# zyc-123/InstanceDiff

Measured on AMD Instinct MI355X. Metric: denoising steps/sec (256x256 bs16), higher is better.
Workload: dtype f32; 1 GPU; 256x256 1-ch synthetic, 1000-step reverse chain, batch 16 per GPU, 2 UNet fwd + reverse update per step; global_batch=16, parallelism=replicas x1 (no collective)

## Files before the change

include/idiff.h:

```cpp
#ifndef IDIFF_H
#define IDIFF_H

#include <stdint.h>

#ifdef __cplusplus
extern "C" {
#endif

#define IDIFF_OK 0
#define IDIFF_E_BADARG (-1)
#define IDIFF_E_UNSUPPORTED (-2)
#define IDIFF_E_HIP (-3)

typedef void* idiff_stream_t;

const char* idiff_last_error(void);
int idiff_version(void);
int64_t idiff_launch_count(void);
int idiff_device_info(int* num_cu, int* wave_size, char* arch_name, int arch_name_len);

#define IDIFF_CONV_NORMAL 0
#define IDIFF_CONV_UPSAMPLE2 1
#define IDIFF_CONV_UNSHUFFLE2 2

// ... 36 lines not shown
    const void* wbf16;
    int32_t operands;
} idiff_conv_desc;

int idiff_conv2d_num_tiles(int Hout, int Wout);
int idiff_conv2d_fwd(const idiff_conv_desc* d, idiff_stream_t stream);
#define IDIFF_CONV_ALGO_DIRECT 0
#define IDIFF_CONV_ALGO_WINOGRAD 1
#define IDIFF_CONV_ALGO_STREAM1X1 2
#define IDIFF_CONV_ALGO_WINOGRAD4 3
#define IDIFF_CONV_ALGO_WINOGRAD4H 4
#define IDIFF_CONV_ALGO_X3 5
#define IDIFF_CONV_ALGO_BF16 6
int idiff_conv2d_last_algo(void);
int idiff_conv2d_plan(const idiff_conv_desc* d);
long long idiff_conv1x1_x3_image_bytes(int Cout, int Cin);
int idiff_pack_conv1x1_x3(const float* w, void* image, int Cout, int Cin, idiff_stream_t stream);
int idiff_pack_conv_weight(const float* w, float* wpk, int Cout, int Cin, int ks, idiff_stream_t stream);
int idiff_pack_conv_weight_T(const float* w, float* wpk, int Cout, int Cin, int ks, idiff_stream_t stream);
int idiff_pack_conv_weight_wino(const float* w, float* wwino, int Cout, int Cin, int transpose, idiff_stream_t stream);
int idiff_pack_conv_weight_wino4(const float* w, float* wwino4, int Cout, int Cin, int transpose, idiff_stream_t stream);
long long idiff_conv_weight_bf16_bytes(int Cout, int Cin, int transpose);
int idiff_pack_conv_weight_bf16(const float* w, void* image, int Cout, int Cin, int transpose, idiff_stream_t stream);

int idiff_gn_finalize(const float* stats, int ntiles, int B, int C, int groups, int HW, const float* gamma,
                      const float* beta, const float* film, int64_t film_ld, float eps, float* out_a, float* out_b,
                      float* mean_rstd, idiff_stream_t stream);

int idiff_affine_silu_add(const float* h, int64_t h_bstride, const float* a, const float* b, const float* res,
                          int64_t res_bstride, const float* vec, float* out, int64_t out_bstride, int B, int C, int HW,
// ... 279 lines not shown
```

instancediff_amd/_lib.py:

```python
import ctypes as C
import os
import re

_HERE = os.path.dirname(os.path.abspath(__file__))
LIB_PATH = os.environ.get("IDIFF_LIB") or os.path.join(_HERE, "libidiff_hip.so")
HEADER_PATH = os.path.join(os.path.dirname(_HERE), "include", "idiff.h")

c_f32p = C.c_void_p
c_stream = C.c_void_p


class ConvDesc(C.Structure):
    _fields_ = [
        ("src0", C.c_void_p), ("src1", C.c_void_p),
        ("src0_bstride", C.c_int64), ("src1_bstride", C.c_int64),
        ("C0", C.c_int32), ("C1", C.c_int32),
        ("B", C.c_int32), ("Hin", C.c_int32), ("Win", C.c_int32),
        ("mode", C.c_int32), ("ks", C.c_int32), ("Cout", C.c_int32),
        ("wpk", C.c_void_p), ("bias", C.c_void_p),
        ("pro_a", C.c_void_p), ("pro_b", C.c_void_p),
        ("out", C.c_void_p), ("out_bstride", C.c_int64),
        ("res", C.c_void_p), ("res_bstride", C.c_int64),
        ("vec", C.c_void_p),
        ("aux", C.c_void_p), ("aux_bstride", C.c_int64), ("aux_a", C.c_void_p), ("aux_b", C.c_void_p),
# ... 29 lines not shown


LINEAR_MAX_GROUPS = 16
XATTN_MAX_GROUPS, MEMPROJ_MAX_GROUPS, SCOREMAP_MAX_GROUPS = 8, 4, 4
P, I, I64, F, U64 = C.c_void_p, C.c_int, C.c_int64, C.c_float, C.c_uint64

SIGNATURES = {
    "idiff_last_error": (C.c_char_p, []),
    "idiff_version": (I, []),
    "idiff_launch_count": (I64, []),
    "idiff_device_info": (I, [C.POINTER(I), C.POINTER(I), C.c_char_p, I]),
    "idiff_conv2d_num_tiles": (I, [I, I]),
    "idiff_conv2d_fwd": (I, [C.POINTER(ConvDesc), c_stream]),
    "idiff_conv2d_last_algo": (I, []),
    "idiff_conv2d_plan": (I, [C.POINTER(ConvDesc)]),
    "idiff_pack_conv_weight": (I, [P, P, I, I, I, c_stream]),
    "idiff_pack_conv_weight_T": (I, [P, P, I, I, I, c_stream]),
    "idiff_pack_conv_weight_wino": (I, [P, P, I, I, I, c_stream]),
    "idiff_pack_conv_weight_wino4": (I, [P, P, I, I, I, c_stream]),
    "idiff_conv_weight_bf16_bytes": (C.c_longlong, [I, I, I]),
    "idiff_pack_conv_weight_bf16": (I, [P, P, I, I, I, c_stream]),
    "idiff_conv1x1_x3_image_bytes": (C.c_longlong, [I, I]),
    "idiff_pack_conv1x1_x3": (I, [P, P, I, I, c_stream]),
    "idiff_gn_finalize": (I, [P, I, I, I, I, I, P, P, P, I64, F, P, P, P, c_stream]),
    "idiff_affine_silu_add": (I, [P, I64, P, P, P, I64, P, P, I64, I, I, I, c_stream]),
    "idiff_linear_fwd": (I, [P, I64, P, I64, P, P, I64, P, P, I64, I, I, I, I, I, c_stream]),
    "idiff_linear_t_fwd": (I, [P, I64, P, I64, P, P, I64, P, P, I64, I, I, I, I, I, c_stream]),
    "idiff_linear_t_ln_fwd": (I, [P, I64, P, P, F, P, I64, P, P, I64, P, P, I64, I, I, I, I, c_stream]),
    "idiff_linear_t_grouped_fwd": (I, [C.POINTER(LinearGroup), I, c_stream]),
    "idiff_attn_tokens_grouped_fwd": (I, [C.POINTER(P), C.POINTER(P), C.POINTER(P), C.POINTER(P), I, I, I, I, I, I, F, I64, I64, c_stream]),
# ... 142 lines not shown
```

instancediff_amd/csrc/conv1x1_x3.hip:

```cpp
#include "conv_args.h"
#include "wino_common.h"

using idiff_detail::ConvArgs;

namespace {

typedef unsigned uintx4 __attribute__((ext_vector_type(4)));
typedef __bf16 bf16x8 __attribute__((ext_vector_type(8)));

constexpr int BM = 64, CKB = 32, NT = 256;
constexpr int B_ISTR = 1088;
constexpr int B_KGSTR = 4 * B_ISTR;
constexpr int B_PLSTR = 4 * B_KGSTR;
constexpr int B_BYTES = 3 * B_PLSTR;
constexpr int A_PLSTR = 4 * 64 * 16;
constexpr int A_BYTES = 3 * A_PLSTR;
constexpr int OLD = 256 + 4;
static_assert(32 * OLD * 4 <= B_BYTES, "epilogue tile must fit in the B planes");

__host__ __device__ constexpr unsigned hi16(unsigned u) { return u & 0xffff0000u; }

__device__ __forceinline__ unsigned pack_hi(unsigned odd, unsigned even) { return __builtin_amdgcn_perm(odd, even, 0x07060302u); }

__device__ __forceinline__ void split3(const float (&x)[8], uintx4& p1, uintx4& p2, uintx4& p3) {
// ... 5 lines not shown
        u2[c] = __builtin_bit_cast(unsigned, r1);
        const float r2 = r1 - __builtin_bit_cast(float, hi16(u2[c]));
        u3[c] = __builtin_bit_cast(unsigned, r2);
    }
    p1 = uintx4{pack_hi(u1[1], u1[0]), pack_hi(u1[3], u1[2]), pack_hi(u1[5], u1[4]), pack_hi(u1[7], u1[6])};
    p2 = uintx4{pack_hi(u2[1], u2[0]), pack_hi(u2[3], u2[2]), pack_hi(u2[5], u2[4]), pack_hi(u2[7], u2[6])};
    p3 = uintx4{pack_hi(u3[1], u3[0]), pack_hi(u3[3], u3[2]), pack_hi(u3[5], u3[4]), pack_hi(u3[7], u3[6])};
}

using idiff_wino::scalar_ptr;

__device__ __forceinline__ floatx4 mma(const uintx4& a, const uintx4& b, const floatx4& c) {
    return __builtin_amdgcn_mfma_f32_16x16x32_bf16(__builtin_bit_cast(bf16x8, a), __builtin_bit_cast(bf16x8, b), c, 0, 0, 0);
}

template <bool UNSH>
__global__ __launch_bounds__(NT) __attribute__((amdgpu_waves_per_eu(2, 2))) void conv1x1_x3_kernel(const ConvArgs a, const unsigned short* __restrict__ wx3) {
    extern __shared__ __attribute__((aligned(16))) unsigned char smem_raw[];
    unsigned char* const Bs = smem_raw;
    unsigned char* const As = smem_raw + B_BYTES;
    float* const econst = reinterpret_cast<float*>(smem_raw + B_BYTES + A_BYTES);

    const int tid = threadIdx.x;
    const int lane = tid & 63;
    const int wave = __builtin_amdgcn_readfirstlane(tid >> 6);
    const int n16 = lane & 15, kgl = lane >> 4;

    const unsigned logical = xcd_remap(blockIdx.x, a.total_wg);
    const int cob = logical % a.ncob;
    const int tile = (logical / a.ncob) % a.ntiles;
    const int b = logical / (a.ncob * a.ntiles);
    const int co0 = cob * BM;
    const long long HW = (long long)a.Hout * a.Wout;
    const long long pix0 = (long long)tile * 256;

    {
        const int which = tid >> 6, co = co0 + (tid & 63);
        float v = 0.f;
        if (which == 0 && a.bias) v = a.bias[co];
        if (which == 1 && a.vec) v = a.vec[(long long)b * a.Cout + co];
        if (which == 2 && a.aux) v = a.aux_a[(long long)b * a.Cout + co];
        if (which == 3 && a.aux) v = a.aux_b[(long long)b * a.Cout + co];
        econst[tid] = v;
    }

    const int q = lane, kg = wave;
    const int nchunks = (a.Cin + CKB - 1) / CKB;
    floatx4 xrA[8], xrB[8];
    uintx4 ar[3];
// ... 104 lines not shown
                }
            }
        }
    };
    load_x(xrA, 0);
    load_w(0);
    load_x(xrB, 1);
    int cc = 0;
    for (; cc + 1 < nchunks; cc += 2) {
        chunk(cc, std::integral_constant<int, 0>{});
        chunk(cc + 1, std::integral_constant<int, 1>{});
    }
    if (cc < nchunks) chunk(cc, std::integral_constant<int, 0>{});

    float* const ot = reinterpret_cast<float*>(Bs);
    float* const outb = a.out + (long long)b * a.obs;
    const float* const resb = a.res ? a.res + (long long)b * a.rbs : nullptr;
    const float* const auxb = a.aux ? a.aux + (long long)b * a.abs_ : nullptr;
    auto rows = [&](int mb, auto res_tag, auto aux_tag) {
        constexpr bool RES = decltype(res_tag)::value, AUX = decltype(aux_tag)::value;
        constexpr int STEPS = 32 * 64 / NT;
        floatx4 nres = {0.f, 0.f, 0.f, 0.f}, naux = {0.f, 0.f, 0.f, 0.f};
        auto fetch = [&](int i) {
            const int f = tid + i * NT;
            const int row = mb * 32 + (f >> 6), c4 = (f & 63) * 4;
            const long long o = (long long)(co0 + row) * HW + pix0 + c4;
            if (RES) nres = *reinterpret_cast<const floatx4*>(resb + o);
            if (AUX) naux = *reinterpret_cast<const floatx4*>(auxb + o);
        };
        fetch(0);
        __syncthreads();
#pragma unroll
        for (int mh = 0; mh < 2; ++mh)
#pragma unroll
            for (int j = 0; j < 4; ++j)
#pragma unroll
                for (int r = 0; r < 4; ++r)
                    ot[(mh * 16 + 4 * kgl + r) * OLD + 64 * wave + 16 * j + n16] = mb ? acc[2 + mh][j][r] : acc[mh][j][r];
        __syncthreads();
#pragma unroll
        for (int i = 0; i < STEPS; ++i) {
            const int f = tid + i * NT;
            const int lrow = f >> 6, row = mb * 32 + lrow, c4 = (f & 63) * 4;
            const floatx4 cres = nres, caux = naux;
            if (i + 1 < STEPS) fetch(i + 1);
            floatx4 v = *reinterpret_cast<const floatx4*>(ot + lrow * OLD + c4);
            const float add = econst[row] + econst[BM + row];
            v = floatx4{v.x + add, v.y + add, v.z + add, v.w + add};
            if (RES) v = floatx4{v.x + cres.x, v.y + cres.y, v.z + cres.z, v.w + cres.w};
            if (AUX) {
                const float aa = econst[2 * BM + row], ab = econst[3 * BM + row];
                v = floatx4{v.x + silu_fast(aa * caux.x + ab), v.y + silu_fast(aa * caux.y + ab), v.z + silu_fast(aa * caux.z + ab),
                            v.w + silu_fast(aa * caux.w + ab)};
            }
            *reinterpret_cast<floatx4*>(outb + (long long)(co0 + row) * HW + pix0 + c4) = v;
        }
    };
    auto halves = [&](auto res_tag, auto aux_tag) {
        rows(0, res_tag, aux_tag);
        rows(1, res_tag, aux_tag);
    };
    if (resb) {
        if (auxb) halves(std::true_type{}, std::true_type{});
        else halves(std::true_type{}, std::false_type{});
    } else {
        if (auxb) halves(std::false_type{}, std::true_type{});
        else halves(std::false_type{}, std::false_type{});
    }
}

__global__ void pack_x3_kernel(const float* __restrict__ w, uintx4* __restrict__ out, int Cout, int Cin, int ncob, long long npieces) {
    for (long long i = blockIdx.x * (long long)blockDim.x + threadIdx.x; i < npieces; i += (long long)gridDim.x * blockDim.x) {
        const int co_l = i & 63;
        const int kg = (i >> 6) & 3;
        const int plane = (int)((i >> 8) % 3);
// ... 17 lines not shown
namespace idiff_detail {

bool conv1x1_x3_eligible(const ConvArgs& a, int mode) {
    const long long hw = (long long)a.Hout * a.Wout;
    if (hw % 256 || hw > (1 << 25) || a.Cout % BM || a.Cin % 8 || a.Cin < CKB || a.pro_a || a.stats) return false;
    if (mode == IDIFF_CONV_UNSHUFFLE2)
        return !a.src1 && a.Wout % 4 == 0 && a.Win == 2 * a.Wout && (long long)a.Hin * a.Win <= (1 << 25) && a.bs0 % 4 == 0 &&
               (reinterpret_cast<uintptr_t>(a.src0) & 15) == 0;
    return mode == IDIFF_CONV_NORMAL && a.Hout == 1 && a.C0v % 8 == 0;
}

int launch_conv1x1_x3(const ConvArgs& a, int mode, const void* wx3, hipStream_t st) {
    const size_t lds = B_BYTES + A_BYTES + 4 * BM * sizeof(float);
    static idiff_dyn_lds_cache lds_cache[2];
    {
        hipError_t e = idiff_ensure_dyn_lds(lds_cache[0], reinterpret_cast<const void*>(conv1x1_x3_kernel<false>), lds);
        if (e == hipSuccess) e = idiff_ensure_dyn_lds(lds_cache[1], reinterpret_cast<const void*>(conv1x1_x3_kernel<true>), lds);
        if (e != hipSuccess) IDIFF_FAIL(IDIFF_E_HIP, "conv2d(1x1 x3): hipFuncSetAttribute: %s", hipGetErrorString(e));
    }
    if (mode == IDIFF_CONV_UNSHUFFLE2) hipLaunchKernelGGL(conv1x1_x3_kernel<true>, dim3(a.total_wg), dim3(NT), lds, st, a, static_cast<const unsigned short*>(wx3));
    else hipLaunchKernelGGL(conv1x1_x3_kernel<false>, dim3(a.total_wg), dim3(NT), lds, st, a, static_cast<const unsigned short*>(wx3));
    IDIFF_CHECK_LAUNCH("conv2d_fwd(1x1 x3)");
    return IDIFF_OK;
}

}

extern "C" long long idiff_conv1x1_x3_image_bytes(int Cout, int Cin) {
    return (long long)((Cin + CKB - 1) / CKB) * ((Cout + BM - 1) / BM) * A_BYTES;
}

extern "C" int idiff_pack_conv1x1_x3(const float* w, void* image, int Cout, int Cin, idiff_stream_t stream) {
    IDIFF_CHECK_ARG(w && image && Cout > 0 && Cin > 0, "pack_conv1x1_x3: bad args");
    IDIFF_CHECK_ARG((reinterpret_cast<uintptr_t>(image) & 15) == 0, "pack_conv1x1_x3: image must be 16-byte aligned");
    const int ncob = (Cout + BM - 1) / BM;
    const long long npieces = idiff_conv1x1_x3_image_bytes(Cout, Cin) / 16;
    const int grid = (int)((npieces + 255) / 256 > 4096 ? 4096 : (npieces + 255) / 256);
// ... 5 lines not shown
```

instancediff_amd/csrc/conv_args.h:

```cpp
#pragma once
#include "common.h"

namespace idiff_detail {

struct GnTail {
    const float* gamma;
    const float* beta;
    const float* film;
    long long film_ld;
    float eps;
    int groups;
    float* out_a;
    float* out_b;
    float* mean_rstd;
};

struct ConvArgs {
    const float* src0;
    const float* src1;
    long long bs0, bs1;
    int C0v, C1v;
    int C0r;
    int Cin;
    int B, Hin, Win, Hout, Wout;
// ... 16 lines not shown
    float* stats;
    GnTail gn;
    int tiles_x, ntiles, ncob;
    unsigned total_wg;
};

bool conv_wino_eligible(const ConvArgs& a, int ks, int mode);
int launch_conv_wino(const ConvArgs& a, int mode, hipStream_t st);

long long conv_wino4_items(const ConvArgs& a, int ks, int mode, bool requested = false);
int launch_conv_wino4(const ConvArgs& a, int mode, hipStream_t st);
int launch_conv_wino4h(const ConvArgs& a, int mode, hipStream_t st);

bool conv1x1_x3_eligible(const ConvArgs& a, int mode);
int launch_conv1x1_x3(const ConvArgs& a, int mode, const void* wx3, hipStream_t st);

bool conv_bf16_eligible(const ConvArgs& a, int ks, int mode, const void* wbf16);
int launch_conv_bf16(const ConvArgs& a, int mode, const void* wbf16, hipStream_t st);

}
```

instancediff_amd/csrc/conv_igemm.hip:

```cpp
#include <stdlib.h>

#include <type_traits>

#include "conv_args.h"

using idiff_detail::ConvArgs;

namespace {

typedef float floatx2 __attribute__((ext_vector_type(2)));

template <int KS, int CK, int TWL, int MODE, bool VECW, int MB, int SPEC>
__global__ __launch_bounds__(256) void conv_igemm_kernel(const ConvArgs a) {
    constexpr int BM = 32 * MB;
    constexpr int TW = 1 << TWL;
    constexpr int TH = 256 / TW;
    constexpr int PAD = KS / 2;
    constexpr int TRH = TH + KS - 1;
    constexpr int RS = TW + KS - 1;
    constexpr int PS = TRH * RS;
    constexpr int IN_TILE = ((CK * PS + 3) / 4) * 4;
    constexpr int TAPS = KS * KS;
    constexpr int W_TILE = TAPS * CK * BM;
    constexpr int BUF = IN_TILE + W_TILE;
// ... 497 lines not shown
        }
    }
}

}

static thread_local int g_last_algo = IDIFF_CONV_ALGO_DIRECT;
extern "C" int idiff_conv2d_last_algo(void) { return g_last_algo; }

extern "C" int idiff_conv2d_num_tiles(int Hout, int Wout) {
    const int twl = pick_twl(Wout);
    const int TW = 1 << twl, TH = 256 / TW;
    return ((Wout + TW - 1) / TW) * ((Hout + TH - 1) / TH);
}

static int conv2d_run(const idiff_conv_desc* d, idiff_stream_t stream, const bool plan) {
    IDIFF_CHECK_ARG(d && d->src0 && d->wpk && d->out, "conv2d: null pointer");
    IDIFF_CHECK_ARG(d->B > 0 && d->C0 > 0 && d->Cout > 0 && d->Hin > 0 && d->Win > 0, "conv2d: bad dims");
    IDIFF_CHECK_ARG(d->ks == 1 || d->ks == 3 || d->ks == 7, "conv2d: ks must be 1, 3 or 7 (got %d)", d->ks);
    IDIFF_CHECK_ARG(d->mode >= 0 && d->mode <= 2, "conv2d: bad mode %d", d->mode);
    IDIFF_CHECK_ARG((d->C1 > 0) == (d->src1 != nullptr), "conv2d: src1/C1 mismatch");
    IDIFF_CHECK_ARG(!(d->pro_a && d->C1 > 0), "conv2d: prologue needs a single source");
    IDIFF_CHECK_ARG((d->pro_a == nullptr) == (d->pro_b == nullptr), "conv2d: pro_a/pro_b must both be set");
    IDIFF_CHECK_ARG(!d->aux || (d->aux_a && d->aux_b), "conv2d: aux needs aux_a/aux_b");
    ConvArgs a;
    a.src0 = d->src0;
    a.src1 = d->src1;
    a.bs0 = d->src0_bstride;
    a.bs1 = d->src1_bstride;
    a.B = d->B;
    a.C0r = d->C0;
    a.Hin = d->Hin;
// ... 37 lines not shown
        a.Wout = d->Win / 2;
    } else if (d->mode == IDIFF_CONV_UPSAMPLE2) {
        a.C0v = d->C0;
        a.C1v = d->C1;
        a.Hout = d->Hin * 2;
        a.Wout = d->Win * 2;
    } else {
        a.C0v = d->C0;
        a.C1v = d->C1;
        a.Hout = d->Hin;
        a.Wout = d->Win;
    }
    a.Cin = a.C0v + a.C1v;
    IDIFF_CHECK_ARG(a.bs0 >= (long long)d->C0 * d->Hin * d->Win, "conv2d: src0_bstride too small");
    IDIFF_CHECK_ARG(d->C1 == 0 || a.bs1 >= (long long)d->C1 * d->Hin * d->Win, "conv2d: src1_bstride too small");
    IDIFF_CHECK_ARG(a.obs >= (long long)d->Cout * a.Hout * a.Wout, "conv2d: out_bstride too small");
    int twl = pick_twl(a.Wout);
    const int mb = a.Cout <= 32 ? 1 : 2;
    const bool vecw = (a.Cout % 4 == 0) && ((reinterpret_cast<uintptr_t>(a.wpk) & 15) == 0);
    const bool in16 = (reinterpret_cast<uintptr_t>(a.src0) & 15) == 0 && (reinterpret_cast<uintptr_t>(a.src1) & 15) == 0 && a.bs0 % 4 == 0 &&
                      (!a.src1 || a.bs1 % 4 == 0);
    if (d->ks == 1 && d->mode == IDIFF_CONV_NORMAL && !a.stats && mb == 2 && vecw && in16 && ((long long)a.Hout * a.Wout) % 256 == 0 &&
        a.Wout >= 32) {
        a.Win = a.Wout = a.Hout * a.Wout;
        a.Hin = a.Hout = 1;
        twl = 8;
    }
    const int TW = 1 << twl, TH = 256 / TW;
    const int bm = 32 * mb;
    a.tiles_x = (a.Wout + TW - 1) / TW;
    a.ntiles = a.tiles_x * ((a.Hout + TH - 1) / TH);
    a.ncob = (a.Cout + bm - 1) / bm;
    const long long total = (long long)a.B * a.ntiles * a.ncob;
    IDIFF_CHECK_ARG(total < (1ll << 31), "conv2d: grid too large");
    a.total_wg = (unsigned)total;
    hipStream_t st = (hipStream_t)stream;
    const bool hard = d->algo_request > 0;
    const int req = (hard ? d->algo_request : -d->algo_request) - 1;
    IDIFF_CHECK_ARG(req == -1 || req == IDIFF_CONV_ALGO_DIRECT || req == IDIFF_CONV_ALGO_WINOGRAD || req == IDIFF_CONV_ALGO_WINOGRAD4 ||
                        req == IDIFF_CONV_ALGO_WINOGRAD4H || req == IDIFF_CONV_ALGO_X3 || req == IDIFF_CONV_ALGO_BF16,
                    "conv2d: bad algo_request %d", d->algo_request);
    IDIFF_CHECK_ARG(d->operands == 0 || d->operands == 1, "conv2d: bad operands %d", d->operands);
    {
        const bool reqbf = req == IDIFF_CONV_ALGO_BF16;
        const bool can = idiff_detail::conv_bf16_eligible(a, d->ks, d->mode, d->wbf16);
        IDIFF_CHECK_ARG(!(hard && reqbf) || can, "conv2d: algo_request bf16 but the layer is not a 3x3 that tiles for it (Cout %% 64, C0 / C1 %% 32, "
                        "Hout %% 8, Wout %% 32) or has no bf16 image");
        if (can && (reqbf || (req == -1 && d->operands == 1))) {
            g_last_algo = IDIFF_CONV_ALGO_BF16;
            if (plan) return IDIFF_OK;
            return finalize_after(idiff_detail::launch_conv_bf16(a, d->mode, d->wbf16, st));
        }
    }
    {
        static const bool x3_on = [] {
            const char* e = getenv("IDIFF_X3");
            return !e || atoi(e) != 0;
// ... 70 lines not shown
    }
    IDIFF_CHECK_ARG(d->mode == IDIFF_CONV_NORMAL, "conv2d: ks=7 needs normal mode");
    return finalize_after(dispatch_mb<7, 2, IDIFF_CONV_NORMAL>(a, twl, mb, vecw, st));
}

extern "C" int idiff_conv2d_fwd(const idiff_conv_desc* d, idiff_stream_t stream) { return conv2d_run(d, stream, false); }

extern "C" int idiff_conv2d_plan(const idiff_conv_desc* d) {
    const int keep = g_last_algo;
    const int rc = conv2d_run(d, nullptr, true);
    const int algo = g_last_algo;
    g_last_algo = keep;
    return rc != IDIFF_OK ? rc : algo;
}

static int pack_common(const float* w, float* wpk, int Cout, int Cin, int ks, int tr, idiff_stream_t stream) {
    IDIFF_CHECK_ARG(w && wpk && Cout > 0 && Cin > 0 && ks > 0, "pack_conv_weight: bad args");
    const long long n = (long long)Cout * Cin * ks * ks;
    const int grid = (int)((n + 255) / 256 > 4096 ? 4096 : (n + 255) / 256);
    hipLaunchKernelGGL(pack_weight_kernel, dim3(grid), dim3(256), 0, (hipStream_t)stream, w, wpk, Cout, Cin, ks * ks, tr);
    IDIFF_CHECK_LAUNCH("pack_conv_weight");
    return IDIFF_OK;
}
extern "C" int idiff_pack_conv_weight(const float* w, float* wpk, int Cout, int Cin, int ks, idiff_stream_t stream) {
    return pack_common(w, wpk, Cout, Cin, ks, 0, stream);
}
extern "C" int idiff_pack_conv_weight_T(const float* w, float* wpk, int Cout, int Cin, int ks, idiff_stream_t stream) {
    return pack_common(w, wpk, Cout, Cin, ks, 1, stream);
}
```

instancediff_amd/csrc/conv_select.hip:

```cpp
#include <stdlib.h>

#include "common.h"

namespace {

constexpr int SCK = 8, STH = 8, STW = 32, SRS = STW + 2, SPS = (STH + 2) * SRS;
constexpr int SNL = (SCK * SPS + 255) / 256;

__global__ __launch_bounds__(256) void conv3x3_select_kernel(const float* __restrict__ x, long long xbs, const float* __restrict__ w,
                                                             const float* __restrict__ bias, const int* __restrict__ idx, float* __restrict__ out,
                                                             int C, int H, int W, int tiles_x) {
    extern __shared__ __attribute__((aligned(16))) float smem[];
    float* tile = smem;
    float* wk = smem + SCK * SPS;
    const int tid = threadIdx.x;
    const int b = blockIdx.y;
    const int y0 = (blockIdx.x / tiles_x) * STH, x0 = (blockIdx.x % tiles_x) * STW;
    const int k = idx[b];
    for (int i = tid; i < C * 9; i += 256) wk[i] = w[(long long)k * C * 9 + i];
    const float* xb = x + (long long)b * xbs;
    const int HW = H * W;
    int goff[SNL];
#pragma unroll
    for (int i = 0; i < SNL; ++i) {
// ... 71 lines not shown
#pragma unroll
                for (int ky = 0; ky < 3; ++ky)
#pragma unroll
                    for (int kx = 0; kx < 3; ++kx) {
                        const float wv = wc[ky * 3 + kx];
#pragma unroll
                        for (int j = 0; j < 4; ++j) acc[j] = __builtin_fmaf(d[u][ky][j + kx], wv, acc[j]);
                    }
            }
        }
    }
    const float bv = bias ? bias[k] : 0.f;
    *reinterpret_cast<floatx4*>(out + (long long)b * HW + p) = floatx4{acc.x + bv, acc.y + bv, acc.z + bv, acc.w + bv};
}

__device__ __forceinline__ void select_window(const float* __restrict__ gb, int y, int x, int H, int W, float (&d)[3][6]) {
#pragma unroll
    for (int r = 0; r < 3; ++r) {
        const int yy = y - 1 + r;
#pragma unroll
        for (int c = 0; c < 6; ++c) {
            const int xx = x - 1 + c;
            d[r][c] = (yy >= 0 && yy < H && xx >= 0 && xx < W) ? gb[(long long)yy * W + xx] : 0.f;
        }
    }
}

__global__ __launch_bounds__(256) void conv3x3_select_dgrad_kernel(const float* __restrict__ g, const float* __restrict__ w, const int* __restrict__ idx,
                                                                   float* __restrict__ dx, long long dbs, int C, int H, int W) {
    extern __shared__ __attribute__((aligned(16))) float wk[];
// ... 86 lines not shown
__global__ __launch_bounds__(256) void conv3x3_select_wgrad_reduce_kernel(const float* __restrict__ ws, const int* __restrict__ idx, float* __restrict__ dw,
                                                                          float* __restrict__ db, int B, int ntile, int C, int K) {
    const int i = blockIdx.x * 256 + threadIdx.x, k = blockIdx.y;
    const int PW = C * 9 + 1;
    if (i >= PW) return;
    float acc = 0.f;
    for (int b = 0; b < B; ++b) {
        if (idx[b] != k) continue;
        const float* wb = ws + (long long)b * ntile * PW + i;
        for (int t = 0; t < ntile; ++t) acc += wb[(long long)t * PW];
    }
    if (i < C * 9) dw[(long long)k * C * 9 + i] = acc;
    else if (db) db[k] = acc;
}

}

static int select_bwd_tiles(int H, int W) { return (int)(((long long)H * W + 4 * 256 * SWG_STRIPS - 1) / (4 * 256 * SWG_STRIPS)); }
extern "C" int64_t idiff_conv3x3_select_bwd_ws_floats(int B, int C, int H, int W) { return (int64_t)B * select_bwd_tiles(H, W) * (C * 9 + 1); }
extern "C" int idiff_conv3x3_select_bwd(const float* x, int64_t x_bstride, const float* w, const int32_t* idx, const float* dpred, float* dx,
                                        int64_t dx_bstride, float* dw, float* db, float* ws, int B, int C, int K, int H, int W, idiff_stream_t stream) {
    IDIFF_CHECK_ARG(x && w && idx && dpred && (dx || dw), "conv3x3_select_bwd: null pointer");
    IDIFF_CHECK_ARG(B > 0 && C > 0 && C <= 256 && K > 0 && H > 0 && W > 0 && W % 4 == 0, "conv3x3_select_bwd: bad dims (W %% 4 == 0, C <= 256)");
    IDIFF_CHECK_ARG(x_bstride % 4 == 0 && (reinterpret_cast<uintptr_t>(x) & 15) == 0, "conv3x3_select_bwd: x must have 16-byte rows");
    IDIFF_CHECK_ARG(!dx || (dx_bstride % 4 == 0 && (reinterpret_cast<uintptr_t>(dx) & 15) == 0), "conv3x3_select_bwd: dx must have 16-byte rows");
    IDIFF_CHECK_ARG(!dw || ws, "conv3x3_select_bwd: the weight gradient needs a workspace of idiff_conv3x3_select_bwd_ws_floats() floats");
    hipStream_t st = (hipStream_t)stream;
    const long long HW = (long long)H * W;
    if (dx) {
        hipLaunchKernelGGL(conv3x3_select_dgrad_kernel, dim3((unsigned)((HW / 4 + 255) / 256), B), dim3(256), (size_t)C * 9 * sizeof(float), st, dpred, w, idx, dx,
// ... 38 lines not shown
```

instancediff_amd/models/modules/MSM_degEmb_Unet.py:

```python
import math
import os
import weakref

import torch
import torch.nn as nn

from ... import ops

ARTIFACT_TYPES = ['speckle in OCT', 'speckle in ultra sound', 'noise in cryo-EM image', 'noise in low dose CT',
                  'Gaussian noise in MRI']


def _trunc_normal_(t, std=0.02):
    return nn.init.trunc_normal_(t, std=std, a=-2 * std, b=2 * std)


def _weight_epoch():
    from ... import train_ops
    return train_ops.WEIGHT_EPOCH[0]


class _Prepared:

    def __init__(self):
# ... 400 lines not shown
    bvf = (ln2.bias.detach().double() @ WvT).float().contiguous()
    return wkf, wvf, bvf


class ResBlock(nn.Module):
    def __init__(self, dim_in, dim_out, time_dim, groups=8):
        super().__init__()
        self.dim_in, self.dim_out, self.groups = dim_in, dim_out, groups
        self.mlp = nn.Linear(time_dim, dim_out * 2)
        self.conv1 = nn.Conv2d(dim_in, dim_out, 3, padding=1)
        self.norm1 = nn.GroupNorm(groups, dim_out)
        self.conv2 = nn.Conv2d(dim_out, dim_out, 3, padding=1)
        self.norm2 = nn.GroupNorm(groups, dim_out)
        self.res_conv = nn.Conv2d(dim_in, dim_out, 1) if dim_in != dim_out else nn.Identity()

    def run(self, src0, src1, film, vec=None, out=None):
        B, _, H, W = src0.shape
        Co, G, HW = self.dim_out, self.groups, H * W
        h1, ab1 = ops.conv2d(src0, packed(self.conv1), self.conv1.bias, 3, Co, src1=src1,
                             gn=dict(groups=G, gamma=self.norm1.weight, beta=self.norm1.bias, film=film, eps=self.norm1.eps))
        h2, (a2, b2) = ops.conv2d(h1, packed(self.conv2), self.conv2.bias, 3, Co, pro=ab1,
                                  gn=dict(groups=G, gamma=self.norm2.weight, beta=self.norm2.bias, eps=self.norm2.eps))
        if isinstance(self.res_conv, nn.Identity):
            assert src1 is None
            return ops.affine_silu_add(h2, (a2, b2), res=src0, vec=vec, out=out)
        return ops.conv2d(src0, packed(self.res_conv), self.res_conv.bias, 1, Co, src1=src1, aux=(h2, a2, b2), vec=vec, out=out)


class ChanLayerNorm(nn.Module):
    def __init__(self, dim):
        super().__init__()
        self.weight = nn.Parameter(torch.ones(dim))
        self.bias = nn.Parameter(torch.zeros(dim))


class CrossAttention(nn.Module):

    def __init__(self, dim, ctx_dim, num_heads=4):
        super().__init__()
        self.dim, self.num_heads = dim, num_heads
# ... 312 lines not shown
            pred.record_stream(cur)
            return (pred, sms) if self.text_module == "scoremap" else pred
        return self._decode(x, x_, hs, films, vecs if single else None, general, ctx, idx, sms if self.text_module == "scoremap" else None)

    def _decode(self, x, x_, hs, films, vecs, general, ctx, idx, sms=None):
        def ca_vec(ca_name, holder):
            return vecs[id(getattr(holder, ca_name))] if vecs is not None else None
        for up in self.ups:
            x = up.res1.run(x, hs.pop(), films[id(up.res1)], vec=ca_vec("ca1", up))
            if general:
                x = up.ca1.run(x, ctx)
            x = up.res2.run(x, hs.pop(), films[id(up.res2)], vec=ca_vec("ca2", up))
            if general:
                x = up.ca2.run(x, ctx)
            x = up.up.run(x)
        x = self.final_res.run(x, x_, films[id(self.final_res)])
        pred = ops.conv3x3_select(x, self.final_conv.weight.detach(), self.final_conv.bias, idx)
        if self.text_module == "scoremap" and sms is not None:
            return pred, sms
        return pred
```

instancediff_amd/ops.py:

```python
import contextlib
import ctypes as C
import math
import os
import threading

import torch

from . import _lib
from ._lib import ConvDesc, check

CONV_NORMAL, CONV_UPSAMPLE2, CONV_UNSHUFFLE2 = 0, 1, 2
ACT_NONE, ACT_SILU, ACT_GELU = 0, 1, 2
SDE_STEP, SDE_MEAN, SDE_ODE = 0, 1, 2

PROFILE = None
ALGO_TRACE = None
WGRAD_TRACE = None


def launch_count():
    return int(_lib.load().idiff_launch_count())


def _stream():
# ... 584 lines not shown
    check(lib.idiff_time_mlp_fwd(_p(t), _p(freqs), _p(w0), _p(b0), _p(w2), _p(b2), _p(out), B, dim, hid, nout, _stream()), "time_mlp")
    return out


def conv3x3_select(x, weight, bias, idx):
    lib = _lib.load()
    B, Cc, H, W = x.shape
    K = weight.shape[0]
    assert tuple(weight.shape) == (K, Cc, 3, 3) and idx.dtype == torch.int32 and idx.numel() == B
    out = torch.empty((B, 1, H, W), device=x.device, dtype=torch.float32)
    check(lib.idiff_conv3x3_select_fwd(_p(x), _bs(x, "x"), _p(_c(weight)), _p(_c(bias)), C.c_void_p(idx.contiguous().data_ptr()), _p(out), B, Cc, K, H, W,
                                       _stream()), "conv3x3_select_fwd")
    return out


def scoremap(feat, tv, idx=None):
    lib = _lib.load()
    B, Cc, H, W = feat.shape
    K = tv.shape[1]
    _c(tv, "tv")
    out = torch.empty((B, K, H, W), device=feat.device, dtype=torch.float32)
    sel = None
    if idx is not None:
        _c(idx, "idx", torch.int32)
        sel = torch.empty((B, 1, H, W), device=feat.device, dtype=torch.float32)
    check(lib.idiff_scoremap_fwd(_p(feat), _bs(feat, "feat"), _p(tv), _p(out), _p(idx), _p(sel), B, Cc, H * W, K, _stream()), "scoremap")
    return out, sel


def image_metrics(pred, target):
# ... 370 lines not shown
```

Baseline: 44.04 steps/s.

## Fuse final 1x1 residual conv with per-sample 3x3 select conv via tap planes

Adds a variant of the bf16x3 1x1 conv kernel that, in its epilogue, projects the 64-channel output tile onto the nine taps of the selected 3x3 output filter. It writes nine tap planes instead of the full 64-channel activation, and a small gather kernel then sums the shifted taps and adds the bias to give the prediction. This avoids writing and re-reading the 64-channel full-resolution tensor before the final select conv. The cost is extra LDS work and syncs in the conv epilogue, a 9-plane intermediate buffer, and one extra launch.

```diff
diff --git a/include/idiff.h b/include/idiff.h
--- a/include/idiff.h
+++ b/include/idiff.h
@@ -74,6 +74,8 @@
 #define IDIFF_CONV_ALGO_BF16 6
 int idiff_conv2d_last_algo(void);
 int idiff_conv2d_plan(const idiff_conv_desc* d);
+int idiff_conv1x1_select_taps_fwd(const idiff_conv_desc* d, const float* w, const float* bias, const int32_t* idx, int K, float* taps,
+                                  float* pred, idiff_stream_t stream);
 long long idiff_conv1x1_x3_image_bytes(int Cout, int Cin);
 int idiff_pack_conv1x1_x3(const float* w, void* image, int Cout, int Cin, idiff_stream_t stream);
 int idiff_pack_conv_weight(const float* w, float* wpk, int Cout, int Cin, int ks, idiff_stream_t stream);
diff --git a/instancediff_amd/_lib.py b/instancediff_amd/_lib.py
--- a/instancediff_amd/_lib.py
+++ b/instancediff_amd/_lib.py
@@ -67,6 +67,7 @@
     "idiff_conv2d_fwd": (I, [C.POINTER(ConvDesc), c_stream]),
     "idiff_conv2d_last_algo": (I, []),
     "idiff_conv2d_plan": (I, [C.POINTER(ConvDesc)]),
+    "idiff_conv1x1_select_taps_fwd": (I, [C.POINTER(ConvDesc), P, P, P, I, P, P, c_stream]),
     "idiff_pack_conv_weight": (I, [P, P, I, I, I, c_stream]),
     "idiff_pack_conv_weight_T": (I, [P, P, I, I, I, c_stream]),
     "idiff_pack_conv_weight_wino": (I, [P, P, I, I, I, c_stream]),
diff --git a/instancediff_amd/csrc/conv1x1_x3.hip b/instancediff_amd/csrc/conv1x1_x3.hip
--- a/instancediff_amd/csrc/conv1x1_x3.hip
+++ b/instancediff_amd/csrc/conv1x1_x3.hip
@@ -43,8 +43,24 @@
     return __builtin_amdgcn_mfma_f32_16x16x32_bf16(__builtin_bit_cast(bf16x8, a), __builtin_bit_cast(bf16x8, b), c, 0, 0, 0);
 }
 
-template <bool UNSH>
-__global__ __launch_bounds__(NT) __attribute__((amdgpu_waves_per_eu(2, 2))) void conv1x1_x3_kernel(const ConvArgs a, const unsigned short* __restrict__ wx3) {
+struct TapArgs {
+    const float* w;
+    const int* idx;
+    float* taps;
+    long long tbs;
+};
+constexpr int TAPW_LD = 12;
+static_assert(BM * TAPW_LD * 4 <= A_BYTES, "tap weights must fit in the A planes");
+static_assert(9 * OLD * 4 <= B_BYTES, "tap tile must fit in the B planes");
+
+__device__ __forceinline__ TapArgs tap_args() { return TapArgs{nullptr, nullptr, nullptr, 0}; }
+__device__ __forceinline__ TapArgs tap_args(const TapArgs& t) { return t; }
+
+template <bool UNSH, bool TAPS, class... Tap>
+__global__ __launch_bounds__(NT) __attribute__((amdgpu_waves_per_eu(2, 2))) void conv1x1_x3_kernel(const ConvArgs a, const unsigned short* __restrict__ wx3,
+                                                                                                   const Tap... tap) {
+    static_assert(sizeof...(Tap) == (TAPS ? 1 : 0), "TAPS takes one TapArgs");
+    const TapArgs tp = tap_args(tap...);
     extern __shared__ __attribute__((aligned(16))) unsigned char smem_raw[];
     unsigned char* const Bs = smem_raw;
     unsigned char* const As = smem_raw + B_BYTES;
@@ -62,6 +78,8 @@
     const int co0 = cob * BM;
     const long long HW = (long long)a.Hout * a.Wout;
     const long long pix0 = (long long)tile * 256;
+    int ksel = 0;
+    if (TAPS) ksel = tp.idx[b];
 
     {
         const int which = tid >> 6, co = co0 + (tid & 63);
@@ -196,10 +214,14 @@
     if (cc < nchunks) chunk(cc, std::integral_constant<int, 0>{});
 
     float* const ot = reinterpret_cast<float*>(Bs);
-    float* const outb = a.out + (long long)b * a.obs;
+    float* const outb = (!TAPS || a.out) ? a.out + (long long)b * a.obs : nullptr;
     const float* const resb = a.res ? a.res + (long long)b * a.rbs : nullptr;
     const float* const auxb = a.aux ? a.aux + (long long)b * a.abs_ : nullptr;
-    auto rows = [&](int mb, auto res_tag, auto aux_tag) {
+    float* const tapw = reinterpret_cast<float*>(As);
+    float tsum[9];
+#pragma unroll
+    for (int t = 0; t < 9; ++t) tsum[t] = 0.f;
+    auto rows = [&](int mb, auto res_tag, auto aux_tag) __attribute__((always_inline)) {
         constexpr bool RES = decltype(res_tag)::value, AUX = decltype(aux_tag)::value;
         constexpr int STEPS = 32 * 64 / NT;
         floatx4 nres = {0.f, 0.f, 0.f, 0.f}, naux = {0.f, 0.f, 0.f, 0.f};
@@ -210,8 +232,22 @@
             if (RES) nres = *reinterpret_cast<const floatx4*>(resb + o);
             if (AUX) naux = *reinterpret_cast<const floatx4*>(auxb + o);
         };
+        float tw[3] = {0.f, 0.f, 0.f};
+        if (TAPS && mb == 0) {
+            const float* const wk = tp.w + (long long)ksel * (BM * 9);
+#pragma unroll
+            for (int i = 0; i < 3; ++i)
+                if (tid + i * NT < BM * 9) tw[i] = wk[tid + i * NT];
+        }
         fetch(0);
         __syncthreads();
+        if (TAPS && mb == 0) {
+#pragma unroll
+            for (int i = 0; i < 3; ++i) {
+                const int e = tid + i * NT, c = e / 9;
+                if (e < BM * 9) tapw[c * TAPW_LD + (e - c * 9)] = tw[i];
+            }
+        }
 #pragma unroll
         for (int mh = 0; mh < 2; ++mh)
 #pragma unroll
@@ -235,12 +271,36 @@
                 v = floatx4{v.x + silu_fast(aa * caux.x + ab), v.y + silu_fast(aa * caux.y + ab), v.z + silu_fast(aa * caux.z + ab),
                             v.w + silu_fast(aa * caux.w + ab)};
             }
-            *reinterpret_cast<floatx4*>(outb + (long long)(co0 + row) * HW + pix0 + c4) = v;
-        }
-    };
-    auto halves = [&](auto res_tag, auto aux_tag) {
+            if (TAPS) *reinterpret_cast<floatx4*>(ot + lrow * OLD + c4) = v;
+            if (!TAPS || outb) *reinterpret_cast<floatx4*>(outb + (long long)(co0 + row) * HW + pix0 + c4) = v;
+        }
+        if (TAPS) {
+            __syncthreads();
+            const float* const vp = ot + tid;
+            const float* const wp = tapw + mb * 32 * TAPW_LD;
+#pragma unroll 8
+            for (int c = 0; c < 32; ++c) {
+                const float v = vp[c * OLD];
+#pragma unroll
+                for (int t = 0; t < 9; ++t) tsum[t] = __builtin_fmaf(wp[c * TAPW_LD + t], v, tsum[t]);
+            }
+        }
+    };
+    auto halves = [&](auto res_tag, auto aux_tag) __attribute__((always_inline)) {
         rows(0, res_tag, aux_tag);
         rows(1, res_tag, aux_tag);
+        if (TAPS) {
+            __syncthreads();
+#pragma unroll
+            for (int t = 0; t < 9; ++t) ot[t * OLD + tid] = tsum[t];
+            __syncthreads();
+            float* const tb = tp.taps + (long long)b * tp.tbs + pix0;
+#pragma unroll
+            for (int i = 0; i < 3; ++i) {
+                const int f = tid + i * NT, t = f >> 6, c4 = (f & 63) * 4;
+                if (f < 9 * 64) *reinterpret_cast<floatx4*>(tb + (long long)t * HW + c4) = *reinterpret_cast<const floatx4*>(ot + t * OLD + c4);
+            }
+        }
     };
     if (resb) {
         if (auxb) halves(std::true_type{}, std::true_type{});
@@ -288,13 +348,29 @@
     const size_t lds = B_BYTES + A_BYTES + 4 * BM * sizeof(float);
     static idiff_dyn_lds_cache lds_cache[2];
     {
-        hipError_t e = idiff_ensure_dyn_lds(lds_cache[0], reinterpret_cast<const void*>(conv1x1_x3_kernel<false>), lds);
-        if (e == hipSuccess) e = idiff_ensure_dyn_lds(lds_cache[1], reinterpret_cast<const void*>(conv1x1_x3_kernel<true>), lds);
+        hipError_t e = idiff_ensure_dyn_lds(lds_cache[0], reinterpret_cast<const void*>(conv1x1_x3_kernel<false, false>), lds);
+        if (e == hipSuccess) e = idiff_ensure_dyn_lds(lds_cache[1], reinterpret_cast<const void*>(conv1x1_x3_kernel<true, false>), lds);
         if (e != hipSuccess) IDIFF_FAIL(IDIFF_E_HIP, "conv2d(1x1 x3): hipFuncSetAttribute: %s", hipGetErrorString(e));
     }
-    if (mode == IDIFF_CONV_UNSHUFFLE2) hipLaunchKernelGGL(conv1x1_x3_kernel<true>, dim3(a.total_wg), dim3(NT), lds, st, a, static_cast<const unsigned short*>(wx3));
-    else hipLaunchKernelGGL(conv1x1_x3_kernel<false>, dim3(a.total_wg), dim3(NT), lds, st, a, static_cast<const unsigned short*>(wx3));
+    if (mode == IDIFF_CONV_UNSHUFFLE2) hipLaunchKernelGGL((conv1x1_x3_kernel<true, false>), dim3(a.total_wg), dim3(NT), lds, st, a, static_cast<const unsigned short*>(wx3));
+    else hipLaunchKernelGGL((conv1x1_x3_kernel<false, false>), dim3(a.total_wg), dim3(NT), lds, st, a, static_cast<const unsigned short*>(wx3));
     IDIFF_CHECK_LAUNCH("conv2d_fwd(1x1 x3)");
+    return IDIFF_OK;
+}
+
+int launch_conv1x1_x3_taps(const ConvArgs& a, const void* wx3, const float* wsel, const int* idx, float* taps, hipStream_t st) {
+    if (a.Cout != BM || a.ncob != 1 || !conv1x1_x3_eligible(a, IDIFF_CONV_NORMAL))
+        IDIFF_FAIL(IDIFF_E_UNSUPPORTED, "conv1x1_select_taps: needs Cout == 64 and a 1x1 layer the bf16x3 kernel takes (got Cout %d)", a.Cout);
+    IDIFF_CHECK_ARG(wsel && idx && taps && (reinterpret_cast<uintptr_t>(taps) & 15) == 0, "conv1x1_select_taps: null pointer, or taps not 16-byte aligned");
+    const size_t lds = B_BYTES + A_BYTES + 4 * BM * sizeof(float);
+    static idiff_dyn_lds_cache lds_cache;
+    {
+        const hipError_t e = idiff_ensure_dyn_lds(lds_cache, reinterpret_cast<const void*>(conv1x1_x3_kernel<false, true, TapArgs>), lds);
+        if (e != hipSuccess) IDIFF_FAIL(IDIFF_E_HIP, "conv1x1_select_taps: hipFuncSetAttribute: %s", hipGetErrorString(e));
+    }
+    const TapArgs tp{wsel, idx, taps, 9ll * a.Hout * a.Wout};
+    hipLaunchKernelGGL((conv1x1_x3_kernel<false, true, TapArgs>), dim3(a.total_wg), dim3(NT), lds, st, a, static_cast<const unsigned short*>(wx3), tp);
+    IDIFF_CHECK_LAUNCH("conv1x1_select_taps(1x1 x3)");
     return IDIFF_OK;
 }
 
diff --git a/instancediff_amd/csrc/conv_args.h b/instancediff_amd/csrc/conv_args.h
--- a/instancediff_amd/csrc/conv_args.h
+++ b/instancediff_amd/csrc/conv_args.h
@@ -54,6 +54,8 @@
 
 bool conv1x1_x3_eligible(const ConvArgs& a, int mode);
 int launch_conv1x1_x3(const ConvArgs& a, int mode, const void* wx3, hipStream_t st);
+int launch_conv1x1_x3_taps(const ConvArgs& a, const void* wx3, const float* wsel, const int* idx, float* taps, hipStream_t st);
+int launch_select_taps_sum(const float* taps, const float* bias, const int* idx, float* pred, int B, int H, int W, hipStream_t st);
 
 bool conv_bf16_eligible(const ConvArgs& a, int ks, int mode, const void* wbf16);
 int launch_conv_bf16(const ConvArgs& a, int mode, const void* wbf16, hipStream_t st);
diff --git a/instancediff_amd/csrc/conv_igemm.hip b/instancediff_amd/csrc/conv_igemm.hip
--- a/instancediff_amd/csrc/conv_igemm.hip
+++ b/instancediff_amd/csrc/conv_igemm.hip
@@ -535,8 +535,16 @@
     return ((Wout + TW - 1) / TW) * ((Hout + TH - 1) / TH);
 }
 
-static int conv2d_run(const idiff_conv_desc* d, idiff_stream_t stream, const bool plan) {
-    IDIFF_CHECK_ARG(d && d->src0 && d->wpk && d->out, "conv2d: null pointer");
+namespace {
+struct SelectTaps {
+    const float* w;
+    const int* idx;
+    float* taps;
+};
+}
+
+static int conv2d_run(const idiff_conv_desc* d, idiff_stream_t stream, const bool plan, const SelectTaps* sel = nullptr) {
+    IDIFF_CHECK_ARG(d && d->src0 && d->wpk && (d->out || sel), "conv2d: null pointer");
     IDIFF_CHECK_ARG(d->B > 0 && d->C0 > 0 && d->Cout > 0 && d->Hin > 0 && d->Win > 0, "conv2d: bad dims");
     IDIFF_CHECK_ARG(d->ks == 1 || d->ks == 3 || d->ks == 7, "conv2d: ks must be 1, 3 or 7 (got %d)", d->ks);
     IDIFF_CHECK_ARG(d->mode >= 0 && d->mode <= 2, "conv2d: bad mode %d", d->mode);
@@ -604,7 +612,7 @@
     a.Cin = a.C0v + a.C1v;
     IDIFF_CHECK_ARG(a.bs0 >= (long long)d->C0 * d->Hin * d->Win, "conv2d: src0_bstride too small");
     IDIFF_CHECK_ARG(d->C1 == 0 || a.bs1 >= (long long)d->C1 * d->Hin * d->Win, "conv2d: src1_bstride too small");
-    IDIFF_CHECK_ARG(a.obs >= (long long)d->Cout * a.Hout * a.Wout, "conv2d: out_bstride too small");
+    IDIFF_CHECK_ARG(!d->out || a.obs >= (long long)d->Cout * a.Hout * a.Wout, "conv2d: out_bstride too small");
     int twl = pick_twl(a.Wout);
     const int mb = a.Cout <= 32 ? 1 : 2;
     const bool vecw = (a.Cout % 4 == 0) && ((reinterpret_cast<uintptr_t>(a.wpk) & 15) == 0);
@@ -631,6 +639,13 @@
                         req == IDIFF_CONV_ALGO_WINOGRAD4H || req == IDIFF_CONV_ALGO_X3 || req == IDIFF_CONV_ALGO_BF16,
                     "conv2d: bad algo_request %d", d->algo_request);
     IDIFF_CHECK_ARG(d->operands == 0 || d->operands == 1, "conv2d: bad operands %d", d->operands);
+    if (sel) {
+        if (d->ks != 1 || d->mode != IDIFF_CONV_NORMAL || twl != 8 || want_gn || d->wx3 == nullptr || (reinterpret_cast<uintptr_t>(d->wx3) & 15) != 0 ||
+            !(req == -1 || req == IDIFF_CONV_ALGO_X3))
+            IDIFF_FAIL(IDIFF_E_UNSUPPORTED, "conv1x1_select_taps: not a flattened 1x1 layer with a split weight image (pixels %% 256, Wout >= 32, 16-byte rows)");
+        g_last_algo = IDIFF_CONV_ALGO_X3;
+        return idiff_detail::launch_conv1x1_x3_taps(a, d->wx3, sel->w, sel->idx, sel->taps, st);
+    }
     {
         const bool reqbf = req == IDIFF_CONV_ALGO_BF16;
         const bool can = idiff_detail::conv_bf16_eligible(a, d->ks, d->mode, d->wbf16);
@@ -731,6 +746,16 @@
     return rc != IDIFF_OK ? rc : algo;
 }
 
+extern "C" int idiff_conv1x1_select_taps_fwd(const idiff_conv_desc* d, const float* w, const float* bias, const int32_t* idx, int K, float* taps,
+                                             float* pred, idiff_stream_t stream) {
+    IDIFF_CHECK_ARG(d && w && idx && taps && pred && K > 0, "conv1x1_select_taps: null pointer");
+    const SelectTaps sel{w, idx, taps};
+    const int H = d->Hin, W = d->Win;
+    const int rc = conv2d_run(d, stream, false, &sel);
+    if (rc != IDIFF_OK) return rc;
+    return idiff_detail::launch_select_taps_sum(taps, bias, idx, pred, d->B, H, W, (hipStream_t)stream);
+}
+
 static int pack_common(const float* w, float* wpk, int Cout, int Cin, int ks, int tr, idiff_stream_t stream) {
     IDIFF_CHECK_ARG(w && wpk && Cout > 0 && Cin > 0 && ks > 0, "pack_conv_weight: bad args");
     const long long n = (long long)Cout * Cin * ks * ks;
diff --git a/instancediff_amd/csrc/conv_select.hip b/instancediff_amd/csrc/conv_select.hip
--- a/instancediff_amd/csrc/conv_select.hip
+++ b/instancediff_amd/csrc/conv_select.hip
@@ -1,6 +1,6 @@
 #include <stdlib.h>
 
-#include "common.h"
+#include "conv_args.h"
 
 namespace {
 
@@ -109,6 +109,25 @@
     *reinterpret_cast<floatx4*>(out + (long long)b * HW + p) = floatx4{acc.x + bv, acc.y + bv, acc.z + bv, acc.w + bv};
 }
 
+__global__ __launch_bounds__(256) void select_taps_sum_kernel(const float* __restrict__ taps, const float* __restrict__ bias, const int* __restrict__ idx,
+                                                              float* __restrict__ out, int H, int W) {
+    const int b = blockIdx.y;
+    const long long HW = (long long)H * W;
+    const long long p = (long long)blockIdx.x * 256 + threadIdx.x;
+    if (p >= HW) return;
+    const int y = (int)(p / W), x = (int)(p - (long long)y * W);
+    const float* tb = taps + (long long)b * 9 * HW + p;
+    float acc = 0.f;
+#pragma unroll
+    for (int t = 0; t < 9; ++t) {
+        const int dy = t / 3 - 1, dx = t % 3 - 1;
+        const bool in = y + dy >= 0 && y + dy < H && x + dx >= 0 && x + dx < W;
+        const float v = in ? tb[(long long)t * HW + dy * W + dx] : 0.f;
+        acc += v;
+    }
+    out[(long long)b * HW + p] = acc + (bias ? bias[idx[b]] : 0.f);
+}
+
 __device__ __forceinline__ void select_window(const float* __restrict__ gb, int y, int x, int H, int W, float (&d)[3][6]) {
 #pragma unroll
     for (int r = 0; r < 3; ++r) {
@@ -225,6 +244,15 @@
     else if (db) db[k] = acc;
 }
 
+}
+
+namespace idiff_detail {
+int launch_select_taps_sum(const float* taps, const float* bias, const int* idx, float* pred, int B, int H, int W, hipStream_t st) {
+    const long long HW = (long long)H * W;
+    hipLaunchKernelGGL(select_taps_sum_kernel, dim3((unsigned)((HW + 255) / 256), B), dim3(256), 0, st, taps, bias, idx, pred, H, W);
+    IDIFF_CHECK_LAUNCH("select_taps_sum");
+    return IDIFF_OK;
+}
 }
 
 static int select_bwd_tiles(int H, int W) { return (int)(((long long)H * W + 4 * 256 * SWG_STRIPS - 1) / (4 * 256 * SWG_STRIPS)); }
diff --git a/instancediff_amd/models/modules/MSM_degEmb_Unet.py b/instancediff_amd/models/modules/MSM_degEmb_Unet.py
--- a/instancediff_amd/models/modules/MSM_degEmb_Unet.py
+++ b/instancediff_amd/models/modules/MSM_degEmb_Unet.py
@@ -438,7 +438,7 @@
         self.norm2 = nn.GroupNorm(groups, dim_out)
         self.res_conv = nn.Conv2d(dim_in, dim_out, 1) if dim_in != dim_out else nn.Identity()
 
-    def run(self, src0, src1, film, vec=None, out=None):
+    def run(self, src0, src1, film, vec=None, out=None, select=None):
         B, _, H, W = src0.shape
         Co, G, HW = self.dim_out, self.groups, H * W
         h1, ab1 = ops.conv2d(src0, packed(self.conv1), self.conv1.bias, 3, Co, src1=src1,
@@ -447,7 +447,11 @@
                                   gn=dict(groups=G, gamma=self.norm2.weight, beta=self.norm2.bias, eps=self.norm2.eps))
         if isinstance(self.res_conv, nn.Identity):
             assert src1 is None
-            return ops.affine_silu_add(h2, (a2, b2), res=src0, vec=vec, out=out)
+            x = ops.affine_silu_add(h2, (a2, b2), res=src0, vec=vec, out=out)
+            return x if select is None else ops.conv3x3_select(x, *select)
+        if select is not None:
+            assert out is None
+            return ops.res_conv_select(src0, src1, packed(self.res_conv), self.res_conv.bias, Co, (h2, a2, b2), vec, *select)
         return ops.conv2d(src0, packed(self.res_conv), self.res_conv.bias, 1, Co, src1=src1, aux=(h2, a2, b2), vec=vec, out=out)
 
 
@@ -790,8 +794,7 @@
             if general:
                 x = up.ca2.run(x, ctx)
             x = up.up.run(x)
-        x = self.final_res.run(x, x_, films[id(self.final_res)])
-        pred = ops.conv3x3_select(x, self.final_conv.weight.detach(), self.final_conv.bias, idx)
+        pred = self.final_res.run(x, x_, films[id(self.final_res)], select=(self.final_conv.weight.detach(), self.final_conv.bias, idx))
         if self.text_module == "scoremap" and sms is not None:
             return pred, sms
         return pred
diff --git a/instancediff_amd/ops.py b/instancediff_amd/ops.py
--- a/instancediff_amd/ops.py
+++ b/instancediff_amd/ops.py
@@ -622,6 +622,66 @@
     return out
 
 
+SELECT_TAPS = bool(int(os.environ.get("IDIFF_SELECT_TAPS", "1")))
+
+
+def select_taps_eligible(src0, src1, wpk, Cout):
+    _, C0, H, W = src0.shape
+    C1 = src1.shape[1] if src1 is not None else 0
+    srcs = [src0] + ([src1] if src1 is not None else [])
+    return (Cout == 64 and getattr(wpk, "x3", None) is not None and (H * W) % 256 == 0 and W >= 32 and C0 % 8 == 0 and C1 % 8 == 0
+            and C0 + C1 >= 32 and all(s.data_ptr() % 16 == 0 and _bs(s, "src") % 4 == 0 for s in srcs))
+
+
+def res_conv_select(src0, src1, wpk, bias, Cout, aux, vec, sel_weight, sel_bias, idx, out=None):
+    if not (SELECT_TAPS and select_taps_eligible(src0, src1, wpk, Cout)):
+        x = conv2d(src0, wpk, bias, 1, Cout, src1=src1, aux=aux, vec=vec, out=out)
+        return conv3x3_select(x, sel_weight, sel_bias, idx)
+    lib = _lib.load()
+    B, C0, H, W = src0.shape
+    K = sel_weight.shape[0]
+    assert tuple(sel_weight.shape) == (K, Cout, 3, 3) and idx.dtype == torch.int32 and idx.numel() == B
+    d = ConvDesc()
+    d.src0, d.src0_bstride, d.C0 = src0.data_ptr(), _bs(src0, "src0"), C0
+    if src1 is not None:
+        assert src1.shape[0] == B and src1.shape[2:] == src0.shape[2:]
+        d.src1, d.src1_bstride, d.C1 = src1.data_ptr(), _bs(src1, "src1"), src1.shape[1]
+    d.B, d.Hin, d.Win, d.mode, d.ks, d.Cout = B, H, W, CONV_NORMAL, 1, Cout
+    d.wpk, d.wx3 = _c(wpk, "wpk").data_ptr(), wpk.x3.data_ptr()
+    if bias is not None:
+        d.bias = _c(bias, "bias").data_ptr()
+    if vec is not None:
+        assert tuple(vec.shape) == (B, Cout)
+        d.vec = _c(vec, "vec").data_ptr()
+    if aux is not None:
+        t, a, b = aux
+        assert tuple(t.shape) == (B, Cout, H, W)
+        d.aux, d.aux_bstride = t.data_ptr(), _bs(t, "aux")
+        d.aux_a, d.aux_b = _c(a, "aux_a").data_ptr(), _c(b, "aux_b").data_ptr()
+    if out is not None:
+        assert tuple(out.shape) == (B, Cout, H, W)
+        d.out, d.out_bstride = out.data_ptr(), _bs(out, "out")
+    taps = torch.empty((B, 9, H, W), device=src0.device, dtype=torch.float32)
+    pred = torch.empty((B, 1, H, W), device=src0.device, dtype=torch.float32)
+
+    def run():
+        check(lib.idiff_conv1x1_select_taps_fwd(C.byref(d), _p(_c(sel_weight)), _p(_c(sel_bias)), C.c_void_p(idx.contiguous().data_ptr()), K, _p(taps),
+                                                _p(pred), _stream()), "conv1x1_select_taps_fwd")
+    if PROFILE is not None:
+        e0, e1 = torch.cuda.Event(enable_timing=True), torch.cuda.Event(enable_timing=True)
+        e0.record()
+        run()
+        e1.record()
+        Cin = C0 + (src1.shape[1] if src1 is not None else 0)
+        PROFILE.append(dict(ks=1, mode=CONV_NORMAL, Cin=Cin, Cout=Cout, B=B, Hout=H, Wout=W, e0=e0, e1=e1, algo=CONV_ALGO_X3,
+                            flops=2.0 * Cin * Cout * H * W * B))
+    else:
+        run()
+    if ALGO_TRACE is not None:
+        ALGO_TRACE[(CONV_ALGO_X3, 1, C0 + (src1.shape[1] if src1 is not None else 0), Cout, H, W)] += 1
+    return pred
+
+
 def scoremap(feat, tv, idx=None):
     lib = _lib.load()
     B, Cc, H, W = feat.shape
```

New measurement: 44.46 steps/s, median of 6. No clear change (+1.0%).
